# lucadellalib/ts-asr

Hardware: AMD Instinct MI355X
Metric: utterance-frames/sec (conformer-t_scratch training step, T=1000, B=32/GPU) (higher is better)
Workload: dtype bf16; 1 GPU; BASELINE.json configs[1]: conformer-t_scratch 12L d256 (+6L speaker encoder), mel [32,1000,80] + enrollment mel [32,500,80] + tokens [32,120], injection cat, dropout 0.1, lens 1.0; global_batch=32, grad_accumulation_factor=1, parallelism=dp1, hip_graph=True

## Files before the change

### ts-asr_amd/csrc/lstm.hip

```cpp
#include <algorithm>

#include <stdlib.h>

#include "common.h"

__device__ __forceinline__ float sigm(float x) { return __builtin_amdgcn_rcpf(1.f + __expf(-x)); }
__device__ __forceinline__ float tanh_fast(float x) { const float e = __expf(-2.f * fabsf(x)); const float t = (1.f - e) * __builtin_amdgcn_rcpf(1.f + e); return x < 0.f ? -t : t; }

template <typename T>
__global__ __launch_bounds__(256) void lstm_cell_fwd_kernel(float *__restrict__ gates, float *__restrict__ c, T *__restrict__ h, int B,
                                                            int U, int H, int t) {
    const int i = blockIdx.x * 256 + threadIdx.x;
    if (i >= B * H) return;
    const int b = i / H, k = i % H;
    float4 *g = reinterpret_cast<float4 *>(gates + (((long long)b * U + t) * H + k) * 4);
    const float4 pre4 = *g;
    const float gi = sigm(pre4.x), gf = sigm(pre4.y), gg = tanh_fast(pre4.z), go = sigm(pre4.w);
    const float cp = t > 0 ? c[((long long)b * U + t - 1) * H + k] : 0.f;
    const float cn = gf * cp + gi * gg;
    *g = make_float4(gi, gf, gg, go);
    c[((long long)b * U + t) * H + k] = cn;
    st1(h + ((long long)b * U + t) * H + k, go * tanh_fast(cn));
}

// ... 388 lines not shown
        if (tid == 0) __hip_atomic_fetch_add(ctr, 1u, __ATOMIC_RELAXED, __HIP_MEMORY_SCOPE_AGENT);
#pragma unroll
        for (int k = 0; k < NST; ++k) {
            const int ch = tid + 256 * k, bl = ch >> 4, part = ch & 15;
            if (ch < BR * 16 && b0 + bl < B)
                *reinterpret_cast<u32x4 *>(dgates + ((long long)(b0 + bl) * U + t) * K4 + (part >> 2) * H + u0 + (part & 3) * 8) = dv16[k];
        }
    }
#ifdef LQ_PROFILE
    if (tid == 0 && wg == 3 && bg == 0) for (int i = 0; i < 5; ++i) reinterpret_cast<long long *>(sync + 32)[i] = bacc_t[i];
#endif
    if (failed && tid == 0) dgates[((long long)min(b0, B - 1) * U) * K4 + u0] = (bf16_t)__builtin_nanf("");
}

#define LQ1_SPINS (1u << 21)
#define LQ1_WGS 16
typedef unsigned short u16x2_t __attribute__((ext_vector_type(2)));
__device__ __forceinline__ unsigned pk_umax16(unsigned a, unsigned b) {
    return __builtin_bit_cast(unsigned, __builtin_elementwise_max(__builtin_bit_cast(u16x2_t, a), __builtin_bit_cast(u16x2_t, b)));
}
__device__ __forceinline__ bool has_unwritten(u32x4 v) {
    const unsigned m = pk_umax16(pk_umax16(v.x, v.y), pk_umax16(v.z, v.w));
    return (m & 0xFFFFu) == 0xFFFFu || m >= 0xFFFF0000u;
}
__device__ __forceinline__ float lane_value(float v, int l) { return __builtin_bit_cast(float, __builtin_amdgcn_readlane(__builtin_bit_cast(int, v), l)); }

__global__ void fill_words_kernel(unsigned *p, size_t n, unsigned v) {
    for (size_t i = blockIdx.x * (size_t)blockDim.x + threadIdx.x; i < n; i += (size_t)gridDim.x * blockDim.x) p[i] = v;
}

#ifdef LQ_PROFILE
#define LQ1_INIT() long long q_acc[4] = {0, 0, 0, 0}, q_prev = clock64()
#define LQ1_STAMP(i) do { const long long n_ = clock64(); q_acc[i] += n_ - q_prev; q_prev = n_; } while (0)
#define LQ1_DUMP() do { if (tid == 0 && blockIdx.x == 24) for (int i = 0; i < 4; ++i) reinterpret_cast<long long *>(sync + 32)[i] = q_acc[i]; } while (0)
#else
#define LQ1_INIT()
#define LQ1_STAMP(i)
#define LQ1_DUMP()
#endif
__device__ __forceinline__ bool lq1_same_xcd(unsigned *ids, int w, int *flag_lds) {
    if (threadIdx.x == 0) {
        const unsigned mine = (__builtin_amdgcn_s_getreg((3 << 11) | (0 << 6) | 20) & 0xFu) + 1u;
        __hip_atomic_store(ids + 2 * w, mine, __ATOMIC_RELAXED, __HIP_MEMORY_SCOPE_AGENT);
        bool same = true;
        for (int i = 0; i < LQ1_WGS && same; ++i) {
            unsigned v = 0, spins = 0;
            while ((v = __hip_atomic_load(ids + 2 * i, __ATOMIC_RELAXED, __HIP_MEMORY_SCOPE_AGENT)) == 0u && ++spins < (1u << 20)) __builtin_amdgcn_s_sleep(1);
            same = (v == mine);
        }
        *flag_lds = same ? 1 : 0;
    }
    __syncthreads();
    return *flag_lds != 0;
}

__device__ __forceinline__ bool lq1_poll_row(const __amdgpu_buffer_rsrc_t rs, int byte_off, u32x4 &row) {
    unsigned spins = 0;
    for (;;) {
        asm volatile("" ::: "memory");
        row = __builtin_amdgcn_raw_buffer_load_b128(rs, byte_off, 0, 16);
        if (__builtin_amdgcn_ballot_w64(has_unwritten(row)) == 0) return true;
        if (++spins > LQ1_SPINS) return false;
    }
}

template <int H>
__global__ __launch_bounds__(384, 1) void lstm_seq1_fwd_kernel(float *__restrict__ gates , float *__restrict__ c , bf16_t *h ,
                                                               const bf16_t *__restrict__ whh , unsigned *sync, int U) {
    static_assert(H == 512 && H == LQ1_WGS * 32, "one 16-byte piece of h_{t-1} per lane; 16 workgroups x 4 waves x 8 units");
    constexpr int KS2 = H / 32;
    if (blockIdx.x & 7) return;
    __shared__ __attribute__((aligned(16))) bf16_t hbuf[2][H];
    __shared__ __attribute__((aligned(16))) float gxr[4][32 * 4];
    __shared__ int fail_flag;
    const int tid = threadIdx.x, lane = tid & 63, wave = tid >> 6, m16 = lane & 15, kg = lane >> 4;
    const int ub = (blockIdx.x >> 3) * 32;
    const __amdgpu_buffer_rsrc_t rs = __builtin_amdgcn_make_buffer_rsrc(h, 0, U * H * 2, 0x00020000);
    if (tid == 0) fail_flag = 0;
    __shared__ int same_flag;
    const bool one_l2 = lq1_same_xcd(sync + 32, blockIdx.x >> 3, &same_flag);
    if (wave == 5) {
        const int l32 = lane & 31;
        auto row = [&](int t) { return *reinterpret_cast<const float4 *>(gates + ((long long)min(t, U - 1) * H + ub + l32) * 4); };
        const float4 a0 = row(0);
        float4 r[4] = {row(1), row(2), row(3), row(4)};
        if (lane < 32) *reinterpret_cast<float4 *>(&gxr[0][l32 * 4]) = a0;
        __syncthreads();
#pragma unroll 1
        for (int t = 1; t < U; t += 4) {
#pragma unroll
            for (int k = 0; k < 4; ++k) {
                const int tt = t + k;
                if (tt < U) {
                    if (lane < 32) *reinterpret_cast<float4 *>(&gxr[tt & 3][l32 * 4]) = r[k];
                    r[k] = row(tt + 4);
                    __syncthreads();
                    if (fail_flag) return;
                }
            }
        }
        return;
    }
    __syncthreads();
    if (wave == 4) {
#pragma unroll 1
        for (int t = 1; t < U; ++t) {
            u32x4 row;
            if (lq1_poll_row(rs, ((t - 1) * H + 8 * lane) * 2, row)) *reinterpret_cast<u32x4 *>(hbuf[t & 1] + 8 * lane) = row;
            else if (lane == 0) fail_flag = 1;
            __syncthreads();
            if (fail_flag) break;
        }
        if (fail_flag && lane == 0) __hip_atomic_store(sync + 1, 1u, __ATOMIC_RELAXED, __HIP_MEMORY_SCOPE_AGENT);
        return;
    }
    const int u0 = ub + 8 * wave;
    bf16x8 af[2][KS2];
#pragma unroll
    for (int rb = 0; rb < 2; ++rb) {
        const bf16_t *wrow = whh + ((long long)(m16 & 3) * H + u0 + 4 * rb + (m16 >> 2)) * H;
#pragma unroll
        for (int s = 0; s < KS2; ++s) af[rb][s] = *reinterpret_cast<const bf16x8 *>(wrow + 32 * s + 8 * kg);
    }
    const int rbl = m16 & 1, ulane = 8 * wave + 4 * rbl + kg;
    float cprev = 0.f;
    LQ1_INIT();
#pragma unroll 1
    for (int t = 0; t < U; ++t) {
        f32x4 acc[2] = {{0.f, 0.f, 0.f, 0.f}, {0.f, 0.f, 0.f, 0.f}};
        LQ1_STAMP(3);
        if (t > 0) {
            __syncthreads();
            if (fail_flag) break;
        }
        LQ1_STAMP(0);
        const float4 gx = *reinterpret_cast<const float4 *>(&gxr[t & 3][ulane * 4]);
        if (t > 0) {
            const bf16_t *hb = hbuf[t & 1];
#pragma unroll
            for (int s = 0; s < KS2; ++s) {
                const bf16x8 b = *reinterpret_cast<const bf16x8 *>(hb + 32 * s + 8 * kg);
                acc[0] = __builtin_amdgcn_mfma_f32_16x16x32_bf16(af[0][s], b, acc[0], 0, 0, 0);
                acc[1] = __builtin_amdgcn_mfma_f32_16x16x32_bf16(af[1][s], b, acc[1], 0, 0, 0);
            }
        }
        const float p0 = rbl ? acc[1][0] : acc[0][0], p1 = rbl ? acc[1][1] : acc[0][1], p2 = rbl ? acc[1][2] : acc[0][2], p3 = rbl ? acc[1][3] : acc[0][3];
        const float gi = sigm(gx.x + p0), gf = sigm(gx.y + p1), gg = tanh_fast(gx.z + p2), go = sigm(gx.w + p3);
        const float cn = gf * cprev + gi * gg;
        cprev = cn;
        const float hv = go * tanh_fast(cn);
        if (m16 < 2) {
            if (one_l2) __builtin_amdgcn_raw_buffer_store_b16(__builtin_bit_cast(unsigned short, (bf16_t)hv), rs, (t * H + ub + ulane) * 2, 0, 0);
            else __builtin_amdgcn_raw_buffer_store_b16(__builtin_bit_cast(unsigned short, (bf16_t)hv), rs, (t * H + ub + ulane) * 2, 0, 16);
            *reinterpret_cast<float4 *>(gates + ((long long)t * H + ub + ulane) * 4) = make_float4(gi, gf, gg, go);
            c[(long long)t * H + ub + ulane] = cn;
        }
        LQ1_STAMP(2);
    }
    LQ1_DUMP();
}

template <int H>
__global__ __launch_bounds__(384, 1) void lstm_seq1_bwd_kernel(const float *__restrict__ gates, const float *__restrict__ c, const bf16_t *__restrict__ dout,
                                                               bf16_t *dgates , const bf16_t *__restrict__ whhT , unsigned *sync, int U) {
    static_assert(H == 512 && H == LQ1_WGS * 32, "four 16-byte pieces of dG_{t+1} per lane; 16 workgroups x 4 waves x 8 units");
    constexpr int K4 = 4 * H, KH = K4 / 2, KS = KH / 32;
    if (blockIdx.x & 7) return;
    __shared__ __attribute__((aligned(16))) bf16_t gbuf[2][K4];
    __shared__ __attribute__((aligned(16))) float opg[4][32 * 4], opc[4][32], opp[4][32];
    __shared__ __attribute__((aligned(16))) bf16_t opd[4][32];
    __shared__ int fail_flag;
    const int tid = threadIdx.x, lane = tid & 63, wave = tid >> 6, m16 = lane & 15, kg = lane >> 4;
    const int ub = (blockIdx.x >> 3) * 32;
    const __amdgpu_buffer_rsrc_t rs = __builtin_amdgcn_make_buffer_rsrc(dgates, 0, U * K4 * 2, 0x00020000);
    if (tid == 0) fail_flag = 0;
    __shared__ int same_flag;
    const bool one_l2 = lq1_same_xcd(sync + 32, blockIdx.x >> 3, &same_flag);
    if (wave == 5) {
        const int l32 = lane & 31;
        auto fetch = [&](int t, float4 &g, float &cn, float &cp, bf16_t &dd) {
            t = max(t, 0);
            g = *reinterpret_cast<const float4 *>(gates + ((long long)t * H + ub + l32) * 4);
            cn = c[(long long)t * H + ub + l32];
            cp = c[(long long)max(t - 1, 0) * H + ub + l32];
            dd = dout[(long long)t * H + ub + l32];
        };
        auto put = [&](int t, const float4 &g, float cn, float cp, bf16_t dd) {
            if (lane < 32) {
                *reinterpret_cast<float4 *>(&opg[t & 3][l32 * 4]) = g;
                opc[t & 3][l32] = cn;
                opp[t & 3][l32] = t > 0 ? cp : 0.f;
                opd[t & 3][l32] = dd;
            }
        };
        float4 g0, g[4]; float cn0, cn[4], cp0, cp[4]; bf16_t d0, d[4];
        fetch(U - 1, g0, cn0, cp0, d0);
#pragma unroll
        for (int k = 0; k < 4; ++k) fetch(U - 2 - k, g[k], cn[k], cp[k], d[k]);
        put(U - 1, g0, cn0, cp0, d0);
        __syncthreads();
#pragma unroll 1
        for (int t = U - 2; t >= 0; t -= 4) {
#pragma unroll
            for (int k = 0; k < 4; ++k) {
                const int tt = t - k;
                if (tt >= 0) {
                    put(tt, g[k], cn[k], cp[k], d[k]);
                    fetch(tt - 4, g[k], cn[k], cp[k], d[k]);
                    __syncthreads();
                    if (fail_flag) return;
                }
            }
        }
        return;
    }
    __syncthreads();
    if (wave == 4) {
#pragma unroll 1
        for (int t = U - 2; t >= 0; --t) {
            u32x4 row[4];
            unsigned spins = 0;
            bool ok = true;
            for (;;) {
                asm volatile("" ::: "memory");
#pragma unroll
                for (int q = 0; q < 4; ++q) row[q] = __builtin_amdgcn_raw_buffer_load_b128(rs, ((t + 1) * K4 + (64 * q + lane) * 8) * 2, 0, 16);
                const bool bad = has_unwritten(row[0]) || has_unwritten(row[1]) || has_unwritten(row[2]) || has_unwritten(row[3]);
                if (__builtin_amdgcn_ballot_w64(bad) == 0) break;
                if (++spins > LQ1_SPINS) { ok = false; break; }
            }
            if (ok) {
#pragma unroll
                for (int q = 0; q < 4; ++q) *reinterpret_cast<u32x4 *>(gbuf[t & 1] + (64 * q + lane) * 8) = row[q];
            } else if (lane == 0) fail_flag = 1;
            __syncthreads();
            if (fail_flag) break;
        }
        if (fail_flag && lane == 0) __hip_atomic_store(sync + 1, 1u, __ATOMIC_RELAXED, __HIP_MEMORY_SCOPE_AGENT);
        return;
    }
    const int uw = ub + 8 * wave;
    bf16x8 af[KS];
    {
        const bf16_t *wrow = whhT + (long long)(uw + (m16 & 7)) * K4 + (m16 >> 3) * KH;
#pragma unroll
        for (int s = 0; s < KS; ++s) af[s] = *reinterpret_cast<const bf16x8 *>(wrow + 32 * s + 8 * kg);
    }
    const int rsel = (m16 >> 1) & 3, ul = 8 * wave + 4 * (kg & 1) + rsel;
    const bool owner = (m16 & 1) == 0 && kg < 2;
    float dcar = 0.f;
    LQ1_INIT();
#pragma unroll 1
    for (int t = U - 1; t >= 0; --t) {
        f32x4 acc = {0.f, 0.f, 0.f, 0.f}, acc2 = {0.f, 0.f, 0.f, 0.f};
        const bool last = (t == U - 1);
        LQ1_STAMP(3);
        if (!last) {
            __syncthreads();
            if (fail_flag) break;
        }
        LQ1_STAMP(0);
        const float4 g4 = *reinterpret_cast<const float4 *>(&opg[t & 3][ul * 4]);
        const float cnv = opc[t & 3][ul], cpv = opp[t & 3][ul], dov = (float)opd[t & 3][ul];
        if (!last) {
            const bf16_t *gb = gbuf[t & 1] + (m16 & 1) * KH + 8 * kg;
#pragma unroll
            for (int s = 0; s < KS; s += 2) {
                acc = __builtin_amdgcn_mfma_f32_16x16x32_bf16(af[s], *reinterpret_cast<const bf16x8 *>(gb + 32 * s), acc, 0, 0, 0);
                acc2 = __builtin_amdgcn_mfma_f32_16x16x32_bf16(af[s + 1], *reinterpret_cast<const bf16x8 *>(gb + 32 * s + 32), acc2, 0, 0, 0);
            }
            acc += acc2;
        }
        const float part = rsel == 0 ? acc[0] : rsel == 1 ? acc[1] : rsel == 2 ? acc[2] : acc[3];
        float other;
        asm volatile("s_nop 1\n\tds_bpermute_b32 %0, %1, %2\n\ts_waitcnt lgkmcnt(0)" : "=&v"(other) : "v"(((lane + 33) & 63) * 4), "v"(part));
        const float dhr = part + other;
        const float gi = g4.x, gf = g4.y, gg = g4.z, go = g4.w;
        const float tc = tanh_fast(cnv);
        const float dh = dov + (last ? 0.f : dhr);
        const float dc = dh * go * (1.f - tc * tc) + dcar;
        const float dgi = dc * gg * gi * (1.f - gi), dgf = dc * cpv * gf * (1.f - gf), dgg = dc * gi * (1.f - gg * gg), dgo = dh * tc * go * (1.f - go);
        dcar = dc * gf;
        if (owner) {
            const int o = (t * K4 + ub + ul) * 2;
            const unsigned short v0 = __builtin_bit_cast(unsigned short, (bf16_t)dgi), v1 = __builtin_bit_cast(unsigned short, (bf16_t)dgf),
                                 v2 = __builtin_bit_cast(unsigned short, (bf16_t)dgg), v3 = __builtin_bit_cast(unsigned short, (bf16_t)dgo);
            if (one_l2) {
                __builtin_amdgcn_raw_buffer_store_b16(v0, rs, o, 0, 0);
                __builtin_amdgcn_raw_buffer_store_b16(v1, rs, o + 2 * H, 0, 0);
                __builtin_amdgcn_raw_buffer_store_b16(v2, rs, o + 4 * H, 0, 0);
                __builtin_amdgcn_raw_buffer_store_b16(v3, rs, o + 6 * H, 0, 0);
            } else {
                __builtin_amdgcn_raw_buffer_store_b16(v0, rs, o, 0, 16);
                __builtin_amdgcn_raw_buffer_store_b16(v1, rs, o + 2 * H, 0, 16);
                __builtin_amdgcn_raw_buffer_store_b16(v2, rs, o + 4 * H, 0, 16);
                __builtin_amdgcn_raw_buffer_store_b16(v3, rs, o + 6 * H, 0, 16);
            }
        }
        LQ1_STAMP(2);
    }
    LQ1_DUMP();
}

static bool lq_seq1(int B, int U, int H) {
    const char *e = getenv("TSASR_LSTM_SEQ1");
    return (!e || e[0] != '0') && B == 1 && H == 512 && (long long)U * 4 * H * 2 < (1ll << 31);
}
static void fill_async(void *p, size_t bytes, unsigned v, hipStream_t st) {
    const size_t n = bytes / 4;
    fill_words_kernel<<<(unsigned)std::min<size_t>(1024, (n + 255) / 256), 256, 0, st>>>((unsigned *)p, n, v);
}

#define LQ_BR 16
static int lq_br(int B) {
    static const int forced = 0;
    if (forced == 8 || forced == 16) return forced;
    return B <= 8 ? 8 : LQ_BR;
}

static int lq_one_xcd() {
    static const int v = [] { const char *e = getenv("TSASR_LSTM_XCD"); return e && e[0] == '1' ? 1 : 0; }();
    return v;
}

__global__ void zero_words_kernel(unsigned *p, size_t n) {
    for (size_t i = blockIdx.x * (size_t)blockDim.x + threadIdx.x; i < n; i += (size_t)gridDim.x * blockDim.x) p[i] = 0u;
}
static void zero_async(void *p, size_t bytes, hipStream_t st) {
    const size_t n = bytes / 4;
    zero_words_kernel<<<(unsigned)std::min<size_t>(1024, (n + 255) / 256), 256, 0, st>>>((unsigned *)p, n);
}

template <int H, int BR>
static void launch_seq_fwd_br(float *gates, float *c, void *h, const void *whh, int B, int U, char *ws, hipStream_t st) {
    auto kern = lstm_seq_fwd_kernel<H, BR>;
    static bool attr = false;
    if (!attr) { (void)hipFuncSetAttribute((const void *)kern, hipFuncAttributeMaxDynamicSharedMemorySize, 96 * 1024); attr = true; }
    zero_async(ws, 256, st);
    const int xcd = lq_one_xcd();
    kern<<<dim3((H / LQ_UN) * (xcd ? 8 : 1), cdiv(B, BR)), 256, 96 * 1024, st>>>(gates, c, (bf16_t *)h, (const bf16_t *)whh, (bf16_t *)(ws + 256), (unsigned *)ws, B, U, xcd);
}
template <int H>
static void launch_seq_fwd(float *gates, float *c, void *h, const void *whh, int B, int U, char *ws, hipStream_t st) {
    if (lq_br(B) == 8) launch_seq_fwd_br<H, 8>(gates, c, h, whh, B, U, ws, st);
    else launch_seq_fwd_br<H, LQ_BR>(gates, c, h, whh, B, U, ws, st);
}
template <int H, int BR>
static void launch_seq_bwd_br(const float *gates, const float *c, const void *dout, void *dgates, const void *whhT, int B, int U, char *ws, hipStream_t st) {
    auto kern = lstm_seq_bwd_kernel<H, BR>;
    static bool attr = false;
    if (!attr) { (void)hipFuncSetAttribute((const void *)kern, hipFuncAttributeMaxDynamicSharedMemorySize, 96 * 1024); attr = true; }
    zero_async(ws, 256, st);
    const int xcd = lq_one_xcd();
    kern<<<dim3((H / LQ_UN) * (xcd ? 8 : 1), cdiv(B, BR)), 256, 96 * 1024, st>>>(gates, c, (const bf16_t *)dout, (bf16_t *)dgates, (const bf16_t *)whhT, (bf16_t *)(ws + 256), (unsigned *)ws, B, U, xcd);
}
template <int H>
static void launch_seq_bwd(const float *gates, const float *c, const void *dout, void *dgates, const void *whhT, int B, int U, char *ws, hipStream_t st) {
    if (lq_br(B) == 8) launch_seq_bwd_br<H, 8>(gates, c, dout, dgates, whhT, B, U, ws, st);
    else launch_seq_bwd_br<H, LQ_BR>(gates, c, dout, dgates, whhT, B, U, ws, st);
}


__global__ __launch_bounds__(256) void lstm_onehot_gates_kernel(const long long *__restrict__ tokens, const float *__restrict__ w_ih,
                                                                 const float *__restrict__ b_ih, const float *__restrict__ b_hh,
                                                                 float *__restrict__ gates, bf16_t *__restrict__ xp, long long BU, int H, int I,
                                                                 int Ip, int blank) {
    const long long n = BU * H;
    for (long long e = (long long)blockIdx.x * 256 + threadIdx.x; e < n; e += (long long)gridDim.x * 256) {
        const long long row = e / H;
        const int h = (int)(e - row * H);
        const long long tok = tokens[row];
        const int col = (tok == blank || tok < 0) ? -1 : (int)(tok > blank ? tok - 1 : tok);
        float v[4];
#pragma unroll
        for (int g = 0; g < 4; ++g) {
            const int k = g * H + h;
            v[g] = b_ih[k] + b_hh[k] + ((col >= 0 && col < I) ? w_ih[(long long)k * I + col] : 0.f);
        }
        *reinterpret_cast<float4 *>(gates + e * 4) = make_float4(v[0], v[1], v[2], v[3]);
        if (xp && h < Ip) xp[row * Ip + h] = (bf16_t)((h == col || h == I || h == I + 1) ? 1.f : 0.f);
    }
}

extern "C" {

int tsasr_lstm_cell_fwd(float *gates, float *c, void *h, int B, int U, int H, int t, int io_dtype, void *stream) {
    TSASR_CHECK_ARG(gates && c && h && B > 0 && U > 0 && H > 0 && t >= 0 && t < U, "tsasr_lstm_cell_fwd: bad arguments");
    const int grid = cdiv(B * H, 256);
    if (io_dtype == TSASR_F32) lstm_cell_fwd_kernel<float><<<grid, 256, 0, (hipStream_t)stream>>>(gates, c, (float *)h, B, U, H, t);
    else if (io_dtype == TSASR_BF16) lstm_cell_fwd_kernel<bf16_t><<<grid, 256, 0, (hipStream_t)stream>>>(gates, c, (bf16_t *)h, B, U, H, t);
    else TSASR_CHECK_ARG(false, "bad io_dtype %d", io_dtype);
    TSASR_CHECK_LAUNCH("tsasr_lstm_cell_fwd");
    return 0;
}

int tsasr_lstm_cell_bwd(const float *gates, const float *c, const void *dout, const float *dh_rec, float *dc_io, void *dgates, int B,
                        int U, int H, int t, int io_dtype, void *stream) {
    TSASR_CHECK_ARG(gates && c && dout && dh_rec && dc_io && dgates && B > 0 && U > 0 && H > 0 && t >= 0 && t < U, "tsasr_lstm_cell_bwd: bad arguments");
    const int grid = cdiv(B * H, 256), last = (t == U - 1);
    if (io_dtype == TSASR_F32) lstm_cell_bwd_kernel<float><<<grid, 256, 0, (hipStream_t)stream>>>(gates, c, (const float *)dout, dh_rec, dc_io, (float *)dgates, B, U, H, t, last);
    else if (io_dtype == TSASR_BF16) lstm_cell_bwd_kernel<bf16_t><<<grid, 256, 0, (hipStream_t)stream>>>(gates, c, (const bf16_t *)dout, dh_rec, dc_io, (bf16_t *)dgates, B, U, H, t, last);
    else TSASR_CHECK_ARG(false, "bad io_dtype %d", io_dtype);
    TSASR_CHECK_LAUNCH("tsasr_lstm_cell_bwd");
    return 0;
}

int tsasr_lstm_step_fwd(float *gates, float *c, void *h, const void *whh, int B, int U, int H, int t, int io_dtype, void *stream) {
    TSASR_CHECK_ARG(gates && c && h && whh && B > 0 && U > 0 && H > 0 && H % 16 == 0 && t >= 0 && t < U, "tsasr_lstm_step_fwd: bad arguments (H=%d)", H);
    dim3 grid(H / LS_UN, cdiv(B, 32));
    if (io_dtype == TSASR_BF16) lstm_step_fwd_kernel<bf16_t><<<grid, 256, 0, (hipStream_t)stream>>>(gates, c, (bf16_t *)h, (const bf16_t *)whh, B, U, H, t);
    else if (io_dtype == TSASR_F32) lstm_step_fwd_kernel<float><<<grid, 256, 0, (hipStream_t)stream>>>(gates, c, (float *)h, (const bf16_t *)whh, B, U, H, t);
    else TSASR_CHECK_ARG(false, "bad io_dtype %d", io_dtype);
    TSASR_CHECK_LAUNCH("tsasr_lstm_step_fwd");
    return 0;
}

int tsasr_lstm_step_bwd(const float *gates, const float *c, const void *dout, void *dgates, const void *whhT, float *dc_io, int B, int U,
                        int H, int t, int io_dtype, void *stream) {
    TSASR_CHECK_ARG(gates && c && dout && dgates && whhT && dc_io && B > 0 && U > 0 && H > 0 && H % 16 == 0 && t >= 0 && t < U, "tsasr_lstm_step_bwd: bad arguments");
    dim3 grid(H / LS_UN, cdiv(B, 32));
    if (io_dtype == TSASR_BF16) lstm_step_bwd_kernel<bf16_t><<<grid, 256, 0, (hipStream_t)stream>>>(gates, c, (const bf16_t *)dout, (bf16_t *)dgates, (const bf16_t *)whhT, dc_io, B, U, H, t);
    else if (io_dtype == TSASR_F32) lstm_step_bwd_kernel<float><<<grid, 256, 0, (hipStream_t)stream>>>(gates, c, (const float *)dout, (float *)dgates, (const bf16_t *)whhT, dc_io, B, U, H, t);
    else TSASR_CHECK_ARG(false, "bad io_dtype %d", io_dtype);
    TSASR_CHECK_LAUNCH("tsasr_lstm_step_bwd");
    return 0;
}

size_t tsasr_lstm_seq_workspace_bytes(int B, int U, int H) {
    const size_t G = (size_t)cdiv(B, 32);
    return 256 + align_up(G * U * 32 * 4 * (size_t)H * sizeof(bf16_t), 256) + align_up((size_t)B * H * sizeof(float), 256);
}

static int device_cu_count() {
    static int cached[64] = {0};
    int dev = 0;
    if (hipGetDevice(&dev) != hipSuccess || dev < 0 || dev >= 64) return 0;
    if (!cached[dev]) {
        int n = 0;
        if (hipDeviceGetAttribute(&n, hipDeviceAttributeMultiprocessorCount, dev) != hipSuccess) n = 0;
        cached[dev] = n > 0 ? n : -1;
    }
    return cached[dev] > 0 ? cached[dev] : 0;
}

static bool seq_persistent_ok(int B, int H, int io_dtype) {
    static const int force_off = getenv("TSASR_LSTM_PERSISTENT") ? (atoi(getenv("TSASR_LSTM_PERSISTENT")) == 0) : 0;
    return !force_off && io_dtype == TSASR_BF16 && (H == 256 || H == 512) && cdiv(B, lq_br(B)) <= 16 &&
           cdiv(B, lq_br(B)) * (H / LQ_UN) <= device_cu_count();
}

int tsasr_lstm_onehot_gates(const long long *tokens, const float *w_ih, const float *b_ih, const float *b_hh, float *gates, void *xp, int B,
                            int U, int H, int I, int Ip, int blank, void *stream) {
    TSASR_CHECK_ARG(tokens && w_ih && b_ih && b_hh && gates && B > 0 && U > 0 && H > 0 && I > 0, "tsasr_lstm_onehot_gates: bad arguments");
    TSASR_CHECK_ARG(!xp || (Ip >= I + 2 && Ip <= H), "tsasr_lstm_onehot_gates: need I + 2 <= Ip <= H (I=%d Ip=%d H=%d)", I, Ip, H);
    const long long n = (long long)B * U * H;
    const unsigned grid = (unsigned)std::min<long long>((n + 255) / 256, 4096);
    lstm_onehot_gates_kernel<<<grid, 256, 0, (hipStream_t)stream>>>(tokens, w_ih, b_ih, b_hh, gates, (bf16_t *)xp, (long long)B * U, H, I, Ip, blank);
    TSASR_CHECK_LAUNCH("tsasr_lstm_onehot_gates");
    return 0;
}

int tsasr_lstm_seq_persistent(int B, int H, int io_dtype) { return seq_persistent_ok(B, H, io_dtype) ? 1 : 0; }

int tsasr_lstm_seq_fwd(float *gates, float *c, void *h, const void *whh, int B, int U, int H, int io_dtype, void *workspace,
                       size_t workspace_bytes, void *stream) {
    TSASR_CHECK_ARG(gates && c && h && whh && B > 0 && U > 0 && H > 0 && H % 16 == 0, "tsasr_lstm_seq_fwd: bad arguments (H=%d)", H);
    hipStream_t st = (hipStream_t)stream;
    if (seq_persistent_ok(B, H, io_dtype)) {
        TSASR_CHECK_ARG(workspace && workspace_bytes >= tsasr_lstm_seq_workspace_bytes(B, U, H), "tsasr_lstm_seq_fwd: workspace too small");
        if (lq_seq1(B, U, H)) {
            zero_async(workspace, 256, st);
            fill_async(h, (size_t)U * H * sizeof(bf16_t), 0xFFFFFFFFu, st);
            lstm_seq1_fwd_kernel<512><<<8 * LQ1_WGS, 384, 0, st>>>(gates, c, (bf16_t *)h, (const bf16_t *)whh, (unsigned *)workspace, U);
        } else if (H == 512) launch_seq_fwd<512>(gates, c, h, whh, B, U, (char *)workspace, st);
        else launch_seq_fwd<256>(gates, c, h, whh, B, U, (char *)workspace, st);
        TSASR_CHECK_LAUNCH("tsasr_lstm_seq_fwd");
        return 0;
    }
    for (int t = 0; t < U; ++t) {
        const int rc = tsasr_lstm_step_fwd(gates, c, h, whh, B, U, H, t, io_dtype, stream);
        if (rc) return rc;
    }
    return 0;
}

int tsasr_lstm_seq_bwd(const float *gates, const float *c, const void *dout, void *dgates, const void *whhT, int B, int U, int H,
                       int io_dtype, void *workspace, size_t workspace_bytes, void *stream) {
    TSASR_CHECK_ARG(gates && c && dout && dgates && whhT && B > 0 && U > 0 && H > 0 && H % 16 == 0, "tsasr_lstm_seq_bwd: bad arguments");
    TSASR_CHECK_ARG(workspace && workspace_bytes >= tsasr_lstm_seq_workspace_bytes(B, U, H), "tsasr_lstm_seq_bwd: workspace too small");
    hipStream_t st = (hipStream_t)stream;
    if (seq_persistent_ok(B, H, io_dtype)) {
        if (lq_seq1(B, U, H)) {
            zero_async(workspace, 256, st);
            fill_async(dgates, (size_t)U * 4 * H * sizeof(bf16_t), 0xFFFFFFFFu, st);
            lstm_seq1_bwd_kernel<512><<<8 * LQ1_WGS, 384, 0, st>>>(gates, c, (const bf16_t *)dout, (bf16_t *)dgates, (const bf16_t *)whhT, (unsigned *)workspace, U);
        } else if (H == 512) launch_seq_bwd<512>(gates, c, dout, dgates, whhT, B, U, (char *)workspace, st);
        else launch_seq_bwd<256>(gates, c, dout, dgates, whhT, B, U, (char *)workspace, st);
        TSASR_CHECK_LAUNCH("tsasr_lstm_seq_bwd");
        return 0;
    }
    const size_t G = (size_t)cdiv(B, 32);
    float *dc_io = (float *)((char *)workspace + 256 + align_up(G * U * 32 * 4 * (size_t)H * sizeof(bf16_t), 256));
    zero_async(dc_io, (size_t)B * H * sizeof(float), st);
    for (int t = U - 1; t >= 0; --t) {
        const int rc = tsasr_lstm_step_bwd(gates, c, dout, dgates, whhT, dc_io, B, U, H, t, io_dtype, stream);
        if (rc) return rc;
    }
    return 0;
}

}
```

Baseline: 3.235 million frames/s.

## Add XCD-grouped persistent LSTM sequence kernels for batched H=512

Adds new persistent forward and backward LSTM recurrence kernels for B>=9, H=512. Each batch group of 16 rows is pinned to 16 workgroups on a single XCD (other workgroups exit), so h/dgates exchange can stay in one L2. Dedicated waves prefetch gate/cell operands and poll peer-written rows into LDS, which overlaps loads with MFMA compute. This launches 8x more workgroups than needed, relies on the dispatcher mapping blockIdx to XCDs round-robin, and has spin-wait failure paths.

```diff
diff --git a/ts-asr_amd/csrc/lstm.hip b/ts-asr_amd/csrc/lstm.hip
--- a/ts-asr_amd/csrc/lstm.hip
+++ b/ts-asr_amd/csrc/lstm.hip
@@ -714,6 +714,347 @@
     LQ1_DUMP();
 }
 
+#define LQX_BR 16
+#define LQX_WGS 16
+typedef unsigned int u32x2 __attribute__((ext_vector_type(2)));
+
+__global__ void lqx_prefill_kernel(unsigned *sync, unsigned *out, size_t n) {
+    for (size_t i = blockIdx.x * (size_t)blockDim.x + threadIdx.x; i < n || i < 64; i += (size_t)gridDim.x * blockDim.x) {
+        if (i < 64) sync[i] = 0u;
+        if (i < n) out[i] = 0xFFFFFFFFu;
+    }
+}
+
+__device__ __forceinline__ bool lqx_same_xcd(unsigned *word, int *flag_lds) {
+    if (threadIdx.x == 0) {
+        const unsigned mine = 1u << (__builtin_amdgcn_s_getreg((3 << 11) | (0 << 6) | 20) & 0xFu);
+        const unsigned before = __hip_atomic_fetch_or(word, mine, __ATOMIC_RELAXED, __HIP_MEMORY_SCOPE_AGENT);
+        asm volatile("" ::"v"(before));
+        __hip_atomic_fetch_add(word, 1u << 16, __ATOMIC_RELAXED, __HIP_MEMORY_SCOPE_AGENT);
+        unsigned v = 0, spins = 0;
+        while (((v = __hip_atomic_load(word, __ATOMIC_RELAXED, __HIP_MEMORY_SCOPE_AGENT)) >> 16) < LQX_WGS && ++spins < (1u << 20)) __builtin_amdgcn_s_sleep(1);
+        *flag_lds = (v == ((unsigned)LQX_WGS << 16 | mine)) ? 1 : 0;
+    }
+    __syncthreads();
+    return *flag_lds != 0;
+}
+
+#ifdef LQ_PROFILE
+#define LQX_POLL_INIT() long long pacc[4] = {0, 0, 0, 0}
+#define LQX_POLL_ARG pacc
+#define LQX_POLL_DUMP() do { if (lane == 0 && pw == 1 && blockIdx.x == 24 && blockIdx.y == 0) for (int i = 0; i < 4; ++i) reinterpret_cast<long long *>(sync + 40)[i] = pacc[i]; } while (0)
+#define LQX_DUMP() do { if (tid == 0 && blockIdx.x == 24 && blockIdx.y == 0) for (int i = 0; i < 4; ++i) reinterpret_cast<long long *>(sync + 32)[i] = q_acc[i]; } while (0)
+#else
+#define LQX_POLL_INIT()
+#define LQX_POLL_ARG nullptr
+#define LQX_POLL_DUMP()
+#define LQX_DUMP()
+#endif
+template <int PPR, bool PROBE>
+__device__ __forceinline__ bool lqx_poll_rows(const __amdgpu_buffer_rsrc_t rs, int step_off, int row_stride, int r0, int nrows, int lane, char *tile, int pitch, long long *pf = nullptr) {
+    unsigned spins = 0;
+    long long pt0 = pf ? clock64() : 0;
+    for (const int pr = min(r0 + 7, nrows - 1); PROBE;) {
+        asm volatile("" ::: "memory");
+        bool bad = false;
+#pragma unroll
+        for (int q = 0; q < PPR; ++q) bad |= has_unwritten(__builtin_amdgcn_raw_buffer_load_b128(rs, pr * row_stride + step_off + (64 * q + lane) * 16, 0, 16));
+        if (__builtin_amdgcn_ballot_w64(bad) == 0) break;
+        if (++spins > LQ1_SPINS) return false;
+    }
+    if (pf) { const long long n_ = clock64(); pf[0] += n_ - pt0; pf[2] += spins + 1; pt0 = n_; }
+    u32x4 v[4][2 * PPR];
+    unsigned pending = 0xFu;
+    for (;;) {
+        asm volatile("" ::: "memory");
+#pragma unroll
+        for (int ch = 0; ch < 4; ++ch)
+            if (pending & (1u << ch)) {
+#pragma unroll
+                for (int k = 0; k < 2 * PPR; ++k)
+                    v[ch][k] = __builtin_amdgcn_raw_buffer_load_b128(rs, min(r0 + 2 * ch + k / PPR, nrows - 1) * row_stride + step_off + (64 * (k % PPR) + lane) * 16, 0, 16);
+            }
+#pragma unroll
+        for (int ch = 0; ch < 4; ++ch)
+            if (pending & (1u << ch)) {
+                bool bad = false;
+#pragma unroll
+                for (int k = 0; k < 2 * PPR; ++k) bad |= has_unwritten(v[ch][k]);
+                if (__builtin_amdgcn_ballot_w64(bad) == 0) {
+#pragma unroll
+                    for (int k = 0; k < 2 * PPR; ++k) {
+                        const int r = r0 + 2 * ch + k / PPR;
+                        if (r < nrows) *reinterpret_cast<u32x4 *>(tile + r * pitch + (64 * (k % PPR) + lane) * 16) = v[ch][k];
+                    }
+                    pending &= ~(1u << ch);
+                }
+            }
+        if (pf) pf[3] += 1;
+        if (!pending) { if (pf) pf[1] += clock64() - pt0; return true; }
+        if (++spins > LQ1_SPINS) return false;
+    }
+}
+
+template <int H>
+__global__ __launch_bounds__(448, 1) void lstm_seqx_fwd_kernel(float *gates , float *__restrict__ c, bf16_t *h ,
+                                                               const bf16_t *__restrict__ whh , unsigned *sync, int B, int U) {
+    static_assert(H == LQX_WGS * LQ_UN, "16 workgroups x 4 waves x 8 units; one 16-byte piece of a row of h per lane");
+    if ((int)(blockIdx.x & 7) != (int)(blockIdx.y & 7)) return;
+    constexpr int KS2 = H / 32, HP = H + 8;
+    __shared__ __attribute__((aligned(16))) bf16_t hbuf[2][LQX_BR][HP];
+    __shared__ __attribute__((aligned(16))) float gxr[2][LQX_BR][33 * 4];
+    __shared__ __attribute__((aligned(16))) bf16_t hs[4][LQX_BR][8];
+    __shared__ int fail_flag, same_flag;
+    const int tid = threadIdx.x, lane = tid & 63, wave = tid >> 6, m16 = lane & 15, kg = lane >> 4;
+    const int wg = blockIdx.x >> 3, bg = blockIdx.y, u0 = wg * LQ_UN, b0 = bg * LQX_BR, nrows = min(LQX_BR, B - b0);
+    const __amdgpu_buffer_rsrc_t rs = __builtin_amdgcn_make_buffer_rsrc(h + (size_t)b0 * U * H, 0, nrows * U * H * 2, 0x00020000);
+    if (tid == 0) fail_flag = 0;
+    for (int i = tid; i < 2 * LQX_BR * HP / 8; i += 448) reinterpret_cast<u32x4 *>(&hbuf[0][0][0])[i] = (u32x4){0u, 0u, 0u, 0u};
+    const bool one_l2 = lqx_same_xcd(sync + 32 + 2 * bg, &same_flag);
+    if (wave == 6) {
+        auto src = [&](int t, int i) __attribute__((always_inline)) {
+            const int q = lane + 64 * i;
+            return reinterpret_cast<const f32x4 *>(gates + (((long long)min(b0 + (q >> 5), B - 1) * U + min(t, U - 1)) * H + u0 + (q & 31)) * 4);
+        };
+        auto dst = [&](int t, int i) __attribute__((always_inline)) {
+            const int q = lane + 64 * i;
+            return reinterpret_cast<f32x4 *>(&gxr[t & 1][q >> 5][(q & 31) * 4]);
+        };
+        struct row8 { f32x4 a, b, c, d, e, f, g, h; } a0, r0, r1, r2, r3;
+#define LQX_FETCH8(R, T) do { R.a = *src(T, 0); R.b = *src(T, 1); R.c = *src(T, 2); R.d = *src(T, 3); R.e = *src(T, 4); R.f = *src(T, 5); R.g = *src(T, 6); R.h = *src(T, 7); } while (0)
+#define LQX_PUT8(R, T) do { *dst(T, 0) = R.a; *dst(T, 1) = R.b; *dst(T, 2) = R.c; *dst(T, 3) = R.d; *dst(T, 4) = R.e; *dst(T, 5) = R.f; *dst(T, 6) = R.g; *dst(T, 7) = R.h; } while (0)
+#define LQX_FSTEP(K, R) do { const int tt = t + K; if (tt < U) { LQX_PUT8(R, tt); LQX_FETCH8(R, tt + 4); __syncthreads(); if (fail_flag) return; } } while (0)
+        LQX_FETCH8(a0, 0);
+        LQX_FETCH8(r0, 1); LQX_FETCH8(r1, 2); LQX_FETCH8(r2, 3); LQX_FETCH8(r3, 4);
+        LQX_PUT8(a0, 0);
+        __syncthreads();
+#pragma unroll 1
+        for (int t = 1; t < U; t += 4) {
+            LQX_FSTEP(0, r0); LQX_FSTEP(1, r1); LQX_FSTEP(2, r2); LQX_FSTEP(3, r3);
+        }
+        return;
+    }
+    __syncthreads();
+    if (wave >= 4) {
+        const int pw = wave - 4;
+        LQX_POLL_INIT();
+#pragma unroll 1
+        for (int t = 1; t < U; ++t) {
+            if (!lqx_poll_rows<1, false>(rs, (t - 1) * H * 2, U * H * 2, 8 * pw, nrows, lane, reinterpret_cast<char *>(&hbuf[t & 1][0][0]), HP * 2, LQX_POLL_ARG) && lane == 0) fail_flag = 1;
+            __syncthreads();
+            if (fail_flag) break;
+        }
+        LQX_POLL_DUMP();
+        if (fail_flag && lane == 0) __hip_atomic_store(sync + 2 * bg + 1, 1u, __ATOMIC_RELAXED, __HIP_MEMORY_SCOPE_AGENT);
+        return;
+    }
+    bf16x8 af[2][KS2];
+#pragma unroll
+    for (int rb = 0; rb < 2; ++rb) {
+        const bf16_t *wrow = whh + ((long long)(m16 & 3) * H + u0 + 8 * wave + 4 * rb + (m16 >> 2)) * H;
+#pragma unroll
+        for (int s = 0; s < KS2; ++s) af[rb][s] = *reinterpret_cast<const bf16x8 *>(wrow + 32 * s + 8 * kg);
+    }
+    const bool live = m16 < nrows;
+    float cprev[2] = {0.f, 0.f};
+    LQ1_INIT();
+#pragma unroll 1
+    for (int t = 0; t < U; ++t) {
+        if (t > 0) {
+            __syncthreads();
+            if (fail_flag) break;
+        }
+        LQ1_STAMP(0);
+        float4 gx[2];
+#pragma unroll
+        for (int rb = 0; rb < 2; ++rb) gx[rb] = *reinterpret_cast<const float4 *>(&gxr[t & 1][m16][(8 * wave + 4 * rb + kg) * 4]);
+        f32x4 acc[2] = {{0.f, 0.f, 0.f, 0.f}, {0.f, 0.f, 0.f, 0.f}};
+        if (t > 0) {
+            const bf16_t *hb = &hbuf[t & 1][m16][8 * kg];
+#pragma unroll
+            for (int s = 0; s < KS2; ++s) {
+                const bf16x8 bfrag = *reinterpret_cast<const bf16x8 *>(hb + 32 * s);
+                acc[0] = __builtin_amdgcn_mfma_f32_16x16x32_bf16(af[0][s], bfrag, acc[0], 0, 0, 0);
+                acc[1] = __builtin_amdgcn_mfma_f32_16x16x32_bf16(af[1][s], bfrag, acc[1], 0, 0, 0);
+            }
+        }
+        float4 gact[2];
+#pragma unroll
+        for (int j = 0; j < 2; ++j) {
+            const float gi = sigm(gx[j].x + acc[j][0]), gf = sigm(gx[j].y + acc[j][1]), gg = tanh_fast(gx[j].z + acc[j][2]), go = sigm(gx[j].w + acc[j][3]);
+            const float cn = gf * cprev[j] + gi * gg;
+            cprev[j] = cn;
+            const float hv = go * tanh_fast(cn);
+            gact[j] = make_float4(gi, gf, gg, go);
+            hs[wave][m16][4 * j + kg] = (bf16_t)hv;
+        }
+        asm volatile("s_waitcnt lgkmcnt(0)" ::: "memory");
+        LQ1_STAMP(1);
+        if (lane < nrows) {
+            const u32x4 hv16 = *reinterpret_cast<const u32x4 *>(&hs[wave][lane][0]);
+            const int off = ((lane * U + t) * H + u0 + 8 * wave) * 2;
+            if (one_l2) __builtin_amdgcn_raw_buffer_store_b128(hv16, rs, off, 0, 0);
+            else __builtin_amdgcn_raw_buffer_store_b128(hv16, rs, off, 0, 16);
+        }
+        asm volatile("s_waitcnt lgkmcnt(0)" ::: "memory");
+        if (live) {
+#pragma unroll
+            for (int j = 0; j < 2; ++j) {
+                const long long e = ((long long)(b0 + m16) * U + t) * H + u0 + 8 * wave + 4 * j + kg;
+                *reinterpret_cast<float4 *>(gates + e * 4) = gact[j];
+                c[e] = cprev[j];
+            }
+        }
+        LQ1_STAMP(2);
+    }
+    LQX_DUMP();
+}
+
+template <int H>
+__global__ __launch_bounds__(512, 1) void lstm_seqx_bwd_kernel(const float *__restrict__ gates, const float *__restrict__ c, const bf16_t *__restrict__ dout,
+                                                               bf16_t *dgates , const bf16_t *__restrict__ whhT ,
+                                                               unsigned *sync, int B, int U) {
+    static_assert(H == LQX_WGS * LQ_UN, "16 workgroups x 32 units; four 16-byte pieces of a row of dgates per lane");
+    if ((int)(blockIdx.x & 7) != (int)(blockIdx.y & 7)) return;
+    constexpr int K4 = 4 * H, XP = K4 + 8, KSW2 = K4 / 32 / 4, SLOT = LQX_BR * LQ_UN;
+    extern __shared__ __attribute__((aligned(16))) char dyn_lds[];
+    bf16_t *xl = reinterpret_cast<bf16_t *>(dyn_lds);
+    float *opg = reinterpret_cast<float *>(dyn_lds + LQX_BR * XP * 2);
+    float *opc = opg + 2 * SLOT * 4, *opp = opc + 2 * SLOT;
+    bf16_t *opd = reinterpret_cast<bf16_t *>(opp + 2 * SLOT);
+    __shared__ float red[4][LQX_BR][33];
+    __shared__ int fail_flag, same_flag;
+    const int tid = threadIdx.x, lane = tid & 63, wave = tid >> 6, m16 = lane & 15, kg = lane >> 4;
+    const int wg = blockIdx.x >> 3, bg = blockIdx.y, u0 = wg * LQ_UN, b0 = bg * LQX_BR, nrows = min(LQX_BR, B - b0);
+    const __amdgpu_buffer_rsrc_t rs = __builtin_amdgcn_make_buffer_rsrc(dgates + (size_t)b0 * U * K4, 0, nrows * U * K4 * 2, 0x00020000);
+    if (tid == 0) fail_flag = 0;
+    for (int i = tid; i < LQX_BR * XP / 8; i += 512) reinterpret_cast<u32x4 *>(xl)[i] = (u32x4){0u, 0u, 0u, 0u};
+    const bool one_l2 = lqx_same_xcd(sync + 32 + 2 * bg, &same_flag);
+    if (wave >= 6) {
+        const int lw = wave - 6, rc = 8 * lw + (lane >> 3), ul4 = (lane & 7) * 4;
+        struct ops_t { f32x4 g0, g1, g2, g3, cn, cp; u32x2 dd; } o0, r0, r1, r2, r3;
+        auto gsrc = [&](int t, int i) __attribute__((always_inline)) {
+            const int q = lane + 64 * i;
+            return reinterpret_cast<const f32x4 *>(gates + (((long long)min(b0 + 8 * lw + (q >> 5), B - 1) * U + t) * H + u0 + (q & 31)) * 4);
+        };
+        auto gdst = [&](int t, int i) __attribute__((always_inline)) {
+            const int q = lane + 64 * i;
+            return reinterpret_cast<f32x4 *>(opg + ((t & 1) * SLOT + (8 * lw + (q >> 5)) * LQ_UN + (q & 31)) * 4);
+        };
+        auto fetch = [&](int t, ops_t &o) __attribute__((always_inline)) {
+            t = max(t, 0);
+            o.g0 = *gsrc(t, 0); o.g1 = *gsrc(t, 1); o.g2 = *gsrc(t, 2); o.g3 = *gsrc(t, 3);
+            const long long rowb = (long long)min(b0 + rc, B - 1) * U;
+            o.cn = *reinterpret_cast<const f32x4 *>(c + (rowb + t) * H + u0 + ul4);
+            o.cp = *reinterpret_cast<const f32x4 *>(c + (rowb + max(t - 1, 0)) * H + u0 + ul4);
+            o.dd = *reinterpret_cast<const u32x2 *>(dout + (rowb + t) * H + u0 + ul4);
+        };
+        auto put = [&](int t, const ops_t &o) __attribute__((always_inline)) {
+            const int s = (t & 1) * SLOT + rc * LQ_UN + ul4;
+            *gdst(t, 0) = o.g0; *gdst(t, 1) = o.g1; *gdst(t, 2) = o.g2; *gdst(t, 3) = o.g3;
+            *reinterpret_cast<f32x4 *>(opc + s) = o.cn;
+            *reinterpret_cast<f32x4 *>(opp + s) = t > 0 ? o.cp : (f32x4){0.f, 0.f, 0.f, 0.f};
+            *reinterpret_cast<u32x2 *>(opd + s) = o.dd;
+        };
+#define LQX_BSTEP(K, R) do { const int tt = t - K; if (tt >= 0) { put(tt, R); fetch(tt - 4, R); __syncthreads(); if (fail_flag) return; __syncthreads(); } } while (0)
+        fetch(U - 1, o0);
+        fetch(U - 2, r0); fetch(U - 3, r1); fetch(U - 4, r2); fetch(U - 5, r3);
+        put(U - 1, o0);
+        __syncthreads();
+        __syncthreads();
+#pragma unroll 1
+        for (int t = U - 2; t >= 0; t -= 4) {
+            LQX_BSTEP(0, r0); LQX_BSTEP(1, r1); LQX_BSTEP(2, r2); LQX_BSTEP(3, r3);
+        }
+        return;
+    }
+    if (wave >= 4) {
+        const int pw = wave - 4;
+        LQX_POLL_INIT();
+        __syncthreads();
+        __syncthreads();
+#pragma unroll 1
+        for (int t = U - 2; t >= 0; --t) {
+            if (!lqx_poll_rows<4, true>(rs, (t + 1) * K4 * 2, U * K4 * 2, 8 * pw, nrows, lane, dyn_lds, XP * 2, LQX_POLL_ARG) && lane == 0) fail_flag = 1;
+            __syncthreads();
+            if (fail_flag) break;
+            __syncthreads();
+        }
+        LQX_POLL_DUMP();
+        if (fail_flag && lane == 0) __hip_atomic_store(sync + 2 * bg + 1, 1u, __ATOMIC_RELAXED, __HIP_MEMORY_SCOPE_AGENT);
+        return;
+    }
+    bf16x8 af[2][KSW2];
+#pragma unroll
+    for (int rb = 0; rb < 2; ++rb) {
+        const bf16_t *wrow = whhT + (long long)(u0 + 16 * rb + m16) * K4;
+#pragma unroll
+        for (int i = 0; i < KSW2; ++i) {
+            const int cp = 32 * (KSW2 * wave + i) + 8 * kg;
+            af[rb][i] = *reinterpret_cast<const bf16x8 *>(wrow + ((cp & 127) >> 5) * H + (cp >> 7) * 32 + (cp & 31));
+        }
+    }
+    float dcar[2] = {0.f, 0.f};
+    LQ1_INIT();
+#pragma unroll 1
+    for (int t = U - 1; t >= 0; --t) {
+        const bool last = (t == U - 1);
+        __syncthreads();
+        if (fail_flag) break;
+        LQ1_STAMP(0);
+        f32x4 acc[2] = {{0.f, 0.f, 0.f, 0.f}, {0.f, 0.f, 0.f, 0.f}};
+        if (!last) {
+#pragma unroll
+            for (int i = 0; i < KSW2; ++i) {
+                const int cp = 32 * (KSW2 * wave + i) + 8 * kg;
+                const bf16x8 bfrag = *reinterpret_cast<const bf16x8 *>(&xl[m16 * XP + ((cp & 127) >> 5) * H + (cp >> 7) * 32 + (cp & 31)]);
+                acc[0] = __builtin_amdgcn_mfma_f32_16x16x32_bf16(af[0][i], bfrag, acc[0], 0, 0, 0);
+                acc[1] = __builtin_amdgcn_mfma_f32_16x16x32_bf16(af[1][i], bfrag, acc[1], 0, 0, 0);
+            }
+        }
+#pragma unroll
+        for (int rb = 0; rb < 2; ++rb)
+#pragma unroll
+            for (int j = 0; j < 4; ++j) red[wave][m16][16 * rb + 4 * kg + j] = acc[rb][j];
+        LQ1_STAMP(1);
+        __syncthreads();
+        LQ1_STAMP(3);
+        const int s = (t & 1) * SLOT;
+#pragma unroll
+        for (int j = 0; j < 2; ++j) {
+            const int p = tid + 256 * j, bl = p >> 5, ul = p & 31;
+            const float dh_rec = red[0][bl][ul] + red[1][bl][ul] + red[2][bl][ul] + red[3][bl][ul];
+            const float4 g4 = *reinterpret_cast<const float4 *>(opg + (s + p) * 4);
+            const float gi = g4.x, gf = g4.y, gg = g4.z, go = g4.w;
+            const float cnv = opc[s + p], cpv = opp[s + p], dov = (float)opd[s + p];
+            const float tc = tanh_fast(cnv);
+            const float dh = dov + (last ? 0.f : dh_rec);
+            const float dc = dh * go * (1.f - tc * tc) + dcar[j];
+            if (bl < nrows) {
+                const int o = ((bl * U + t) * K4 + u0 + ul) * 2;
+                const unsigned short v0 = __builtin_bit_cast(unsigned short, (bf16_t)(dc * gg * gi * (1.f - gi))),
+                                     v1 = __builtin_bit_cast(unsigned short, (bf16_t)(dc * cpv * gf * (1.f - gf))),
+                                     v2 = __builtin_bit_cast(unsigned short, (bf16_t)(dc * gi * (1.f - gg * gg))),
+                                     v3 = __builtin_bit_cast(unsigned short, (bf16_t)(dh * tc * go * (1.f - go)));
+                if (one_l2) {
+                    __builtin_amdgcn_raw_buffer_store_b16(v0, rs, o, 0, 0);
+                    __builtin_amdgcn_raw_buffer_store_b16(v1, rs, o + 2 * H, 0, 0);
+                    __builtin_amdgcn_raw_buffer_store_b16(v2, rs, o + 4 * H, 0, 0);
+                    __builtin_amdgcn_raw_buffer_store_b16(v3, rs, o + 6 * H, 0, 0);
+                } else {
+                    __builtin_amdgcn_raw_buffer_store_b16(v0, rs, o, 0, 16);
+                    __builtin_amdgcn_raw_buffer_store_b16(v1, rs, o + 2 * H, 0, 16);
+                    __builtin_amdgcn_raw_buffer_store_b16(v2, rs, o + 4 * H, 0, 16);
+                    __builtin_amdgcn_raw_buffer_store_b16(v3, rs, o + 6 * H, 0, 16);
+                }
+            }
+            dcar[j] = dc * gf;
+        }
+        LQ1_STAMP(2);
+    }
+    LQX_DUMP();
+}
+
 static bool lq_seq1(int B, int U, int H) {
     const char *e = getenv("TSASR_LSTM_SEQ1");
     return (!e || e[0] != '0') && B == 1 && H == 512 && (long long)U * 4 * H * 2 < (1ll << 31);
@@ -872,6 +1213,27 @@
     return 0;
 }
 
+static bool lq_groupx(int B, int U, int H) {
+    const char *e = getenv("TSASR_LSTM_GROUPX");
+    const int G = cdiv(B, LQX_BR);
+    return (!e || e[0] != '0') && H == 512 && B >= 9 && G <= 16 && (long long)LQX_BR * U * 4 * H * 2 < (1ll << 31) &&
+           cdiv(G, 8) * LQX_WGS * 8 <= device_cu_count();
+}
+static void launch_seqx_fwd(float *gates, float *c, void *h, const void *whh, int B, int U, char *ws, hipStream_t st) {
+    const size_t n = (size_t)B * U * 512 * sizeof(bf16_t) / 4;
+    lqx_prefill_kernel<<<(unsigned)std::min<size_t>(1024, (n + 255) / 256), 256, 0, st>>>((unsigned *)ws, (unsigned *)h, n);
+    lstm_seqx_fwd_kernel<512><<<dim3(8 * LQX_WGS, cdiv(B, LQX_BR)), 448, 0, st>>>(gates, c, (bf16_t *)h, (const bf16_t *)whh, (unsigned *)ws, B, U);
+}
+static void launch_seqx_bwd(const float *gates, const float *c, const void *dout, void *dgates, const void *whhT, int B, int U, char *ws, hipStream_t st) {
+    constexpr int LDS = LQX_BR * (4 * 512 + 8) * 2 + 2 * LQX_BR * LQ_UN * (16 + 4 + 4 + 2);
+    auto kern = lstm_seqx_bwd_kernel<512>;
+    static bool attr = false;
+    if (!attr) { (void)hipFuncSetAttribute((const void *)kern, hipFuncAttributeMaxDynamicSharedMemorySize, LDS); attr = true; }
+    const size_t n = (size_t)B * U * 4 * 512 * sizeof(bf16_t) / 4;
+    lqx_prefill_kernel<<<(unsigned)std::min<size_t>(1024, (n + 255) / 256), 256, 0, st>>>((unsigned *)ws, (unsigned *)dgates, n);
+    kern<<<dim3(8 * LQX_WGS, cdiv(B, LQX_BR)), 512, LDS, st>>>(gates, c, (const bf16_t *)dout, (bf16_t *)dgates, (const bf16_t *)whhT, (unsigned *)ws, B, U);
+}
+
 int tsasr_lstm_seq_persistent(int B, int H, int io_dtype) { return seq_persistent_ok(B, H, io_dtype) ? 1 : 0; }
 
 int tsasr_lstm_seq_fwd(float *gates, float *c, void *h, const void *whh, int B, int U, int H, int io_dtype, void *workspace,
@@ -884,7 +1246,8 @@
             zero_async(workspace, 256, st);
             fill_async(h, (size_t)U * H * sizeof(bf16_t), 0xFFFFFFFFu, st);
             lstm_seq1_fwd_kernel<512><<<8 * LQ1_WGS, 384, 0, st>>>(gates, c, (bf16_t *)h, (const bf16_t *)whh, (unsigned *)workspace, U);
-        } else if (H == 512) launch_seq_fwd<512>(gates, c, h, whh, B, U, (char *)workspace, st);
+        } else if (lq_groupx(B, U, H)) launch_seqx_fwd(gates, c, h, whh, B, U, (char *)workspace, st);
+        else if (H == 512) launch_seq_fwd<512>(gates, c, h, whh, B, U, (char *)workspace, st);
         else launch_seq_fwd<256>(gates, c, h, whh, B, U, (char *)workspace, st);
         TSASR_CHECK_LAUNCH("tsasr_lstm_seq_fwd");
         return 0;
@@ -906,7 +1269,8 @@
             zero_async(workspace, 256, st);
             fill_async(dgates, (size_t)U * 4 * H * sizeof(bf16_t), 0xFFFFFFFFu, st);
             lstm_seq1_bwd_kernel<512><<<8 * LQ1_WGS, 384, 0, st>>>(gates, c, (const bf16_t *)dout, (bf16_t *)dgates, (const bf16_t *)whhT, (unsigned *)workspace, U);
-        } else if (H == 512) launch_seq_bwd<512>(gates, c, dout, dgates, whhT, B, U, (char *)workspace, st);
+        } else if (lq_groupx(B, U, H)) launch_seqx_bwd(gates, c, dout, dgates, whhT, B, U, (char *)workspace, st);
+        else if (H == 512) launch_seq_bwd<512>(gates, c, dout, dgates, whhT, B, U, (char *)workspace, st);
         else launch_seq_bwd<256>(gates, c, dout, dgates, whhT, B, U, (char *)workspace, st);
         TSASR_CHECK_LAUNCH("tsasr_lstm_seq_bwd");
         return 0;
```

Result: no change. 3.261 million frames/s (median of 3 runs) (+0.8%).
